# ShenhanQian/GaussianAvatars

Measured on AMD Instinct MI355X. Metric: frames/sec fwd+bwd @100k SH-3 splats 802x550, higher is better.
Workload: dtype f32; 1 GPU; BASELINE configs[2]: 100000 mesh-bound SH-3 splats (synthetic stand-in for media/306), 802x550 (HxW), select_mesh_by_timestep + render + L1-vs-white + backward, no optimiser step; splats=100000, width=550, height=802, sh_degree=3, scene=ellipsoid, splat_order=morton (io.spatial_sort: the loaders' default), num_rendered=2322054, num_binned=1851307, tile_culling=True, binding=fused, parallelism=one process, one GPU, 300 frames in turn; no collective

## Files before the change

### gaussianavatars_amd/csrc/gsr_backward.hip

```cpp
#include "gsr_device.h"

#include <hip/amd_detail/amd_hip_unsafe_atomics.h>

namespace gsr {

__device__ __forceinline__ float swap32_add(float a, float b)
{
    const auto r = __builtin_amdgcn_permlane32_swap(__float_as_uint(a), __float_as_uint(b), false, false);
    return __uint_as_float(r[0]) + __uint_as_float(r[1]);
}
__device__ __forceinline__ float swap16_add(float a, float b)
{
    const auto r = __builtin_amdgcn_permlane16_swap(__float_as_uint(a), __float_as_uint(b), false, false);
    return __uint_as_float(r[0]) + __uint_as_float(r[1]);
}
__device__ __forceinline__ float bank_merge(float keep, float take, const int bank_mask_sel)
{
    return bank_mask_sel == 0xA
               ? __int_as_float(__builtin_amdgcn_update_dpp(__float_as_int(keep), __float_as_int(take), 0xE4, 0xf, 0xA, false))
               : __int_as_float(__builtin_amdgcn_update_dpp(__float_as_int(keep), __float_as_int(take), 0xE4, 0xf, 0xC, false));
}
__device__ __forceinline__ float row_sum4(float a, float b, float c, float d)
{
    a += dpp_f<0x141, 0xf>(a);
// ... 358 lines not shown
        const int j = hi - 1 - lane;
        const bool valid = lane < CH && j < nq;
        const uint32_t idx = qp[valid ? j : nq - 1];
        const float4 r0 = grec[3 * (size_t)idx + 0], r1 = grec[3 * (size_t)idx + 1], r2 = grec[3 * (size_t)idx + 2];
        const float xq = r0.x - fqx0, yq = r0.y - fqy0;
        const float cA = r0.z, cB = r0.w, cC = r1.x;
        const float op = valid ? r2.z : 0.f;
        const float cr = r1.z, cgn = r1.w, cb = r2.x;
        const int jrec = valid ? j : 0x7fffffff;
        const unsigned long long act = __ballot(last_pix > lo);
        const bool more = lo > seg_lo;
        f2 a0 = {0.f, 0.f}, a1 = a0, a2 = a0, a3 = a0, a4 = a0, a5 = a0, a6 = a0, a7 = a0, a8 = a0;

        for (int r = 0; r < 8; ++r) {
            const uint32_t rm = (uint32_t)(act >> (8 * r)) & 0xFFu;
            if (!rm) continue;
            const float dy = yq - (float)r;
            const float Bdy = cB * dy, Cdy2 = (cC * dy) * dy;
#ifndef GSR_EXP_NO_ROW_SUMS
            f2 rs0 = {0.f, 0.f}, rs1 = rs0, rs2 = rs0;
#endif
#pragma unroll
            for (int h = 0; h < 2; ++h) {
                if (!((rm >> (4 * h)) & 0xFu)) continue;
                const f4* tp = reinterpret_cast<const f4*>(tab + (r * 4 + 2 * h) * 12);
                f4 t[2][3];
#pragma unroll
                for (int e = 0; e < 2; ++e)
#pragma unroll
                    for (int k = 0; k < 3; ++k) t[e][k] = tp[3 * e + k];
                f2 dx[2], a0m[2], al[2], rv[2], R[2], Tj[2], cg[2], aT[2], Pw[2];
#pragma unroll
                for (int e = 0; e < 2; ++e) {
                    const float c0 = (float)(4 * h + 2 * e);
                    dx[e] = f2{xq - c0, xq - (c0 + 1.0f)};
                    const f2 pw = (cA * dx[e] + Bdy) * dx[e] + Cdy2;
                    const f2 G = {__builtin_amdgcn_exp2f(pw.x), __builtin_amdgcn_exp2f(pw.y)};
                    const f2 araw = op * G;
                    const int l0 = __float_as_int(t[e][2].z), l1 = __float_as_int(t[e][2].w);
#ifdef GSR_EXP_HI_TEST
                    a0m[e].x = (l0 > jrec && pw.x <= 0.0f && araw.x >= 1.0f / 255.0f) ? araw.x : 0.0f;
                    a0m[e].y = (l1 > jrec && pw.y <= 0.0f && araw.y >= 1.0f / 255.0f) ? araw.y : 0.0f;
#else
                    a0m[e].x = (l0 > jrec && araw.x >= 1.0f / 255.0f) ? araw.x : 0.0f;
                    a0m[e].y = (l1 > jrec && araw.y >= 1.0f / 255.0f) ? araw.y : 0.0f;
#endif
                    al[e] = f2{__builtin_fminf(0.99f, a0m[e].x), __builtin_fminf(0.99f, a0m[e].y)};
                    const f2 om = 1.0f - al[e];
                    rv[e] = f2{__builtin_amdgcn_rcpf(om.x), __builtin_amdgcn_rcpf(om.y)};
                    R[e] = rv[e];
                }
#ifndef GSR_EXP_RP_NOSCAN
                GSR_SCAN4("v_mul_f32_dpp", R[0].x, R[0].y, R[1].x, R[1].y);
#endif
#pragma unroll
                for (int e = 0; e < 2; ++e) {
                    const f2 Te = {t[e][0].x, t[e][0].y};
                    const f2 g0 = {t[e][1].x, t[e][1].y}, g1 = {t[e][1].z, t[e][1].w}, g2 = {t[e][2].x, t[e][2].y};
                    Tj[e] = Te * R[e];
                    cg[e] = cr * g0 + (cgn * g1 + cb * g2);
                    aT[e] = al[e] * Tj[e];
                    Pw[e] = aT[e] * cg[e];
                }
#ifndef GSR_EXP_RP_NOSCAN
                GSR_SCAN4("v_add_f32_dpp", Pw[0].x, Pw[0].y, Pw[1].x, Pw[1].y);
#endif
#pragma unroll
                for (int e = 0; e < 2; ++e) {
                    const f2 Sx = {t[e][0].z, t[e][0].w};
                    const f2 g0 = {t[e][1].x, t[e][1].y}, g1 = {t[e][1].z, t[e][1].w}, g2 = {t[e][2].x, t[e][2].y};
                    const f2 dLda = ((Tj[e] * cg[e] - Pw[e]) - Sx) * rv[e];
                    const f2 tq = a0m[e] * dLda;
                    a0 += aT[e] * g0;
                    a1 += aT[e] * g1;
                    a2 += aT[e] * g2;
#ifndef GSR_EXP_NO_ROW_SUMS
                    const f2 ax = tq * dx[e];
                    rs0 += tq;
                    rs1 += ax;
                    rs2 += ax * dx[e];
#else
                    const f2 ax = tq * dx[e], ay = tq * dy;
                    a3 += ax;
                    a4 += ay;
                    a5 += ax * dx[e];
                    a6 += ax * dy;
                    a7 += ay * dy;
                    a8 += tq;
#endif
                    if (more) {
                        const float T0 = __int_as_float(__builtin_amdgcn_readlane(__float_as_int(Tj[e].x), CH - 1));
                        const float T1 = __int_as_float(__builtin_amdgcn_readlane(__float_as_int(Tj[e].y), CH - 1));
                        const float S0 = __int_as_float(__builtin_amdgcn_readlane(__float_as_int(Pw[e].x), CH - 1)) + Sx.x;
                        const float S1 = __int_as_float(__builtin_amdgcn_readlane(__float_as_int(Pw[e].y), CH - 1)) + Sx.y;
                        if (lane == 0) {
                            float* up = tab + (r * 4 + 2 * h + e) * 12;
                            up[0] = T0; up[1] = T1; up[2] = S0; up[3] = S1;
                        }
                    }
                }
            }
#ifndef GSR_EXP_NO_ROW_SUMS
            a3 += rs1;
            a4 += rs0 * dy;
            a5 += rs2;
            a6 += rs1 * dy;
            a7 += rs0 * (dy * dy);
            a8 += rs0;
#endif
        }
#ifndef GSR_EXP_RP_NOATOMIC
        {
            const float v[9] = {a0.x + a0.y, a1.x + a1.y, a2.x + a2.y, a3.x + a3.y, a4.x + a4.y, a5.x + a5.y, a6.x + a6.y, a7.x + a7.y, a8.x + a8.y};
#pragma unroll
            for (int c = 0; c < 9; ++c) xs[9 * lane + c] = v[c];
#pragma unroll
            for (int i = 0; i < (CH + 6) / 7; ++i) {
                const int rl7 = (lane * 7282) >> 16;
                const int c = lane - 9 * rl7;
                const int rl = 7 * i + rl7;
                const float val = xs[63 * i + lane];
                const uint32_t rid = (uint32_t)__builtin_amdgcn_ds_bpermute(rl << 2, (int)idx);
                const bool live = lane < 63 && rl < CH && (hi - 1 - rl) < nq;
#ifdef GSR_EXP_RP_PLAINSTORE
                if (live && val == 12345.678f) acc[(size_t)GSR_ACC_STRIDE * rid + c] = val;
#else
                if (live && val != 0.f) unsafeAtomicAdd(acc + (size_t)GSR_ACC_STRIDE * rid + c, val);
#endif
            }
        }
#endif
        if (!more) break;
        hi = lo;
    }
    }
}

template __global__ void k_render_bwd_rp<1>(Settings, const uint32_t*, const uint32_t*, const float4*, const uint32_t*, const float*, const uint32_t*, const float*, float*, const float*,
                                             const float4*, int, unsigned long long, const unsigned long long*, const uint32_t*);
template __global__ void k_render_bwd_rp<2>(Settings, const uint32_t*, const uint32_t*, const float4*, const uint32_t*, const float*, const uint32_t*, const float*, float*, const float*,
                                             const float4*, int, unsigned long long, const unsigned long long*, const uint32_t*);
template __global__ void k_render_bwd_rp<4>(Settings, const uint32_t*, const uint32_t*, const float4*, const uint32_t*, const float*, const uint32_t*, const float*, float*, const float*,
                                             const float4*, int, unsigned long long, const unsigned long long*, const uint32_t*);


__global__ __launch_bounds__(GSR_PREBWD_ROWS) void k_preprocess_bwd(Settings s, PreBwdArgs a)
{
    const int i = blockIdx.x * blockDim.x + threadIdx.x;
    const int M = a.M;
    __shared__ float sh_lds[GSR_PREBWD_ROWS * GSR_SH_MAX_STRIDE];
    const bool sh_staged = !a.use_precomp_color && a.dL_dsh != nullptr && M <= 16;
    const int first = blockIdx.x * GSR_PREBWD_ROWS, rows = min(GSR_PREBWD_ROWS, a.P - first);
    const int sh_stride = sh_row_stride(M);
    if (sh_staged) {
        if (a.shs_rest) {
            sh_rows_load<GSR_PREBWD_ROWS>(sh_lds, a.shs, first, rows, 3, sh_stride, 0, (int)threadIdx.x);
            sh_rows_load<GSR_PREBWD_ROWS>(sh_lds, a.shs_rest, first, rows, 3 * (M - 1), sh_stride, 3, (int)threadIdx.x);
        } else {
            sh_rows_load<GSR_PREBWD_ROWS>(sh_lds, a.shs, first, rows, 3 * M, sh_stride, 0, (int)threadIdx.x);
        }
        __syncthreads();
    }
    if (i < a.P) {
    float dmean[3] = {0.f, 0.f, 0.f};
    float gcov[6] = {0.f, 0.f, 0.f, 0.f, 0.f, 0.f};
    float dscale[3] = {0.f, 0.f, 0.f};
    float drot[4] = {0.f, 0.f, 0.f, 0.f};
    float gcol[3] = {0.f, 0.f, 0.f};
    float g2x = 0.f, g2y = 0.f, gop = 0.f;
    const bool vis = a.radii[i] > 0;
    float* gsh = a.dL_dsh ? (sh_staged ? sh_lds + (int)threadIdx.x * sh_row_stride(M) : a.dL_dsh + (size_t)3 * M * i) : nullptr;

    if (vis) {
        float4 q0, q1, q2;
        if (s.deterministic) {
            long long* ai = a.acc64 + (size_t)GSR_ACC64_STRIDE * i;
            const int ex = __float_as_int(a.grec[3 * (size_t)i + 2].y), back = gmax_exponent(*a.gmax) - GSR_FIXED_BITS;
            float f[9];
#pragma unroll
            for (int k = 0; k < 9; ++k) { f[k] = __builtin_ldexpf((float)ai[k], back + ((k >= 5 && k <= 7) ? (ex >> 8) : (ex & 0xFF))); ai[k] = 0ll; }
            q0 = make_float4(f[0], f[1], f[2], f[3]); q1 = make_float4(f[4], f[5], f[6], f[7]); q2 = make_float4(f[8], 0.f, 0.f, 0.f);
        } else {
            float4* ac4 = (float4*)(a.acc + (size_t)GSR_ACC_STRIDE * i);
            q0 = ac4[0]; q1 = ac4[1]; q2 = ac4[2];
            const float4 z = make_float4(0.f, 0.f, 0.f, 0.f);
            ac4[0] = z; ac4[1] = z; ac4[2] = z;
        }
        gcol[0] = q0.x; gcol[1] = q0.y; gcol[2] = q0.z;
        g2x = -0.5f * (float)s.W * q0.w; g2y = -0.5f * (float)s.H * q1.x;
        const float gA = -0.5f * q1.y, gB = -0.5f * q1.z, gC = -0.5f * q1.w;
        gop = q2.x;
        const float* vm = s.viewmatrix;
        const float* proj = s.projmatrix;
        const int W = s.W, H = s.H;
        const float fx = (float)W / (2.0f * s.tanfovx), fy = (float)H / (2.0f * s.tanfovy);
        float mx = a.means3D[3 * i], my = a.means3D[3 * i + 1], mz = a.means3D[3 * i + 2];
        if (a.bound.binding) {
            const long long bface = bound_face(a.bound, i);
            float w[3];
            bindm::world_xyz(a.bound.fR + 9 * bface, a.bound.fs[bface], a.bound.fc + 3 * bface, mx, my, mz, w);
            mx = w[0]; my = w[1]; mz = w[2];
        }
        const float* c6 = a.cov3D + 6 * i;

        if (!a.use_precomp_color) {
            float shr[48];
            {
                const float* row = sh_staged ? sh_lds + (int)threadIdx.x * sh_row_stride(M) : a.shs + (size_t)3 * M * i;
#pragma unroll
                for (int k = 0; k < 48; ++k) shr[k] = k < 3 * M ? row[k] : 0.f;
            }
            const float* sh = shr;
            const int deg = s.sh_degree;
            const float d0 = mx - s.campos[0], d1 = my - s.campos[1], d2 = mz - s.campos[2];
            const float sum2 = d0 * d0 + d1 * d1 + d2 * d2;
            const float inv_len = 1.0f / sqrtf(sum2);
            const float x = d0 * inv_len, y = d1 * inv_len, z = d2 * inv_len;
            const uint32_t cl = a.clamped[i];
            float ddir[3] = {0.f, 0.f, 0.f};
            const float xx = x * x, yy = y * y, zz = z * z, xy_ = x * y, yz = y * z, xz = x * z;
            const int ncoef = (deg + 1) * (deg + 1);
#pragma unroll
            for (int c = 0; c < 3; ++c) {
                const float g = ((cl >> c) & 1u) ? 0.f : gcol[c];
                float dxs = 0.f, dys = 0.f, dzs = 0.f;
                gsh[0 + c] = kC0 * g;
                if (deg > 0) {
                    gsh[3 + c] = -kC1 * y * g;
                    gsh[6 + c] = kC1 * z * g;
                    gsh[9 + c] = -kC1 * x * g;
                    dxs = -kC1 * sh[9 + c];
                    dys = -kC1 * sh[3 + c];
                    dzs = kC1 * sh[6 + c];
                    if (deg > 1) {
                        gsh[12 + c] = kC2_0 * xy_ * g;
                        gsh[15 + c] = kC2_1 * yz * g;
                        gsh[18 + c] = kC2_2 * (2.f * zz - xx - yy) * g;
                        gsh[21 + c] = kC2_3 * xz * g;
                        gsh[24 + c] = kC2_4 * (xx - yy) * g;
                        dxs += kC2_0 * y * sh[12 + c] + kC2_2 * 2.f * -x * sh[18 + c] + kC2_3 * z * sh[21 + c] + kC2_4 * 2.f * x * sh[24 + c];
                        dys += kC2_0 * x * sh[12 + c] + kC2_1 * z * sh[15 + c] + kC2_2 * 2.f * -y * sh[18 + c] + kC2_4 * 2.f * -y * sh[24 + c];
                        dzs += kC2_1 * y * sh[15 + c] + kC2_2 * 2.f * 2.f * z * sh[18 + c] + kC2_3 * x * sh[21 + c];
                        if (deg > 2) {
                            gsh[27 + c] = kC3_0 * y * (3.f * xx - yy) * g;
                            gsh[30 + c] = kC3_1 * xy_ * z * g;
                            gsh[33 + c] = kC3_2 * y * (4.f * zz - xx - yy) * g;
                            gsh[36 + c] = kC3_3 * z * (2.f * zz - 3.f * xx - 3.f * yy) * g;
                            gsh[39 + c] = kC3_4 * x * (4.f * zz - xx - yy) * g;
                            gsh[42 + c] = kC3_5 * z * (xx - yy) * g;
                            gsh[45 + c] = kC3_6 * x * (xx - 3.f * yy) * g;
                            dxs += kC3_0 * sh[27 + c] * 3.f * 2.f * xy_ + kC3_1 * sh[30 + c] * yz + kC3_2 * sh[33 + c] * -2.f * xy_ +
                                   kC3_3 * sh[36 + c] * -3.f * 2.f * xz + kC3_4 * sh[39 + c] * (-3.f * xx + 4.f * zz - yy) +
                                   kC3_5 * sh[42 + c] * 2.f * xz + kC3_6 * sh[45 + c] * 3.f * (xx - yy);
                            dys += kC3_0 * sh[27 + c] * 3.f * (xx - yy) + kC3_1 * sh[30 + c] * xz +
                                   kC3_2 * sh[33 + c] * (-3.f * yy + 4.f * zz - xx) + kC3_3 * sh[36 + c] * -3.f * 2.f * yz +
                                   kC3_4 * sh[39 + c] * -2.f * xy_ + kC3_5 * sh[42 + c] * -2.f * yz + kC3_6 * sh[45 + c] * -3.f * 2.f * xy_;
                            dzs += kC3_1 * sh[30 + c] * xy_ + kC3_2 * sh[33 + c] * 4.f * 2.f * yz +
                                   kC3_3 * sh[36 + c] * 3.f * (2.f * zz - xx - yy) + kC3_4 * sh[39 + c] * 4.f * 2.f * xz +
                                   kC3_5 * sh[42 + c] * (xx - yy);
                        }
                    }
                }
                ddir[0] += dxs * g;
                ddir[1] += dys * g;
                ddir[2] += dzs * g;
            }
            for (int k = 3 * ncoef; k < 3 * M; ++k) gsh[k] = 0.f;
            const float invsum32 = 1.0f / sqrtf(sum2 * sum2 * sum2);
            dmean[0] += ((sum2 - d0 * d0) * ddir[0] - d1 * d0 * ddir[1] - d2 * d0 * ddir[2]) * invsum32;
            dmean[1] += (-d0 * d1 * ddir[0] + (sum2 - d1 * d1) * ddir[1] - d2 * d1 * ddir[2]) * invsum32;
            dmean[2] += (-d0 * d2 * ddir[0] - d1 * d2 * ddir[1] + (sum2 - d2 * d2) * ddir[2]) * invsum32;
        }

        float t0 = vm[0] * mx + vm[4] * my + vm[8] * mz + vm[12];
        float t1 = vm[1] * mx + vm[5] * my + vm[9] * mz + vm[13];
        const float t2 = vm[2] * mx + vm[6] * my + vm[10] * mz + vm[14];
        const float limx = 1.3f * s.tanfovx, limy = 1.3f * s.tanfovy;
        const float txtz = t0 / t2, tytz = t1 / t2;
        t0 = sel_min(limx, sel_max(-limx, txtz)) * t2;
        t1 = sel_min(limy, sel_max(-limy, tytz)) * t2;
        const float x_grad_mul = (txtz < -limx || txtz > limx) ? 0.f : 1.f;
        const float y_grad_mul = (tytz < -limy || tytz > limy) ? 0.f : 1.f;
        const float J00 = fx / t2, J02 = -(fx * t0) / (t2 * t2), J11 = fy / t2, J12 = -(fy * t1) / (t2 * t2);
        float A[2][3];
#pragma unroll
        for (int j = 0; j < 3; ++j) {
            A[0][j] = J00 * vm[4 * j + 0] + J02 * vm[4 * j + 2];
            A[1][j] = J11 * vm[4 * j + 1] + J12 * vm[4 * j + 2];
        }
        const float V[3][3] = {{c6[0], c6[1], c6[2]}, {c6[1], c6[3], c6[4]}, {c6[2], c6[4], c6[5]}};
        float AV[2][3];
#pragma unroll
        for (int r = 0; r < 2; ++r)
#pragma unroll
            for (int j = 0; j < 3; ++j) AV[r][j] = A[r][0] * V[0][j] + A[r][1] * V[1][j] + A[r][2] * V[2][j];
        const float ca = AV[0][0] * A[0][0] + AV[0][1] * A[0][1] + AV[0][2] * A[0][2] + 0.3f;
        const float cb = AV[0][0] * A[1][0] + AV[0][1] * A[1][1] + AV[0][2] * A[1][2];
        const float cc = AV[1][0] * A[1][0] + AV[1][1] * A[1][1] + AV[1][2] * A[1][2] + 0.3f;
        const float denom = ca * cc - cb * cb;
        if (s.fast_blend) {
            const float det_inv = 1.f / denom;
            const float kA = cc * det_inv, kB = -cb * det_inv, kC = ca * det_inv;
            g2x = -0.5f * (float)s.W * (kA * q0.w + kB * q1.x);
            g2y = -0.5f * (float)s.H * (kC * q1.x + kB * q0.w);
            const float opac = a.grec[3 * (size_t)i + 2].z;
            gop = opac > 0.f ? q2.x / opac : 0.f;
        }
        const float denom2inv = 1.0f / ((denom * denom) + 0.0000001f);
        float dL_da = 0.f, dL_db = 0.f, dL_dc = 0.f;
        if (denom2inv != 0.f) {
            dL_da = denom2inv * (-cc * cc * gA + 2.f * cb * cc * gB + (denom - ca * cc) * gC);
            dL_dc = denom2inv * (-ca * ca * gC + 2.f * ca * cb * gB + (denom - ca * cc) * gA);
            dL_db = denom2inv * 2.f * (cb * cc * gA - (denom + 2.f * cb * cb) * gB + ca * cb * gC);
            gcov[0] = A[0][0] * A[0][0] * dL_da + A[0][0] * A[1][0] * dL_db + A[1][0] * A[1][0] * dL_dc;
            gcov[3] = A[0][1] * A[0][1] * dL_da + A[0][1] * A[1][1] * dL_db + A[1][1] * A[1][1] * dL_dc;
            gcov[5] = A[0][2] * A[0][2] * dL_da + A[0][2] * A[1][2] * dL_db + A[1][2] * A[1][2] * dL_dc;
            gcov[1] = 2.f * A[0][0] * A[0][1] * dL_da + (A[0][0] * A[1][1] + A[0][1] * A[1][0]) * dL_db + 2.f * A[1][0] * A[1][1] * dL_dc;
            gcov[2] = 2.f * A[0][0] * A[0][2] * dL_da + (A[0][0] * A[1][2] + A[0][2] * A[1][0]) * dL_db + 2.f * A[1][0] * A[1][2] * dL_dc;
            gcov[4] = 2.f * A[0][2] * A[0][1] * dL_da + (A[0][1] * A[1][2] + A[0][2] * A[1][1]) * dL_db + 2.f * A[1][1] * A[1][2] * dL_dc;
        }
        float dA[2][3];
#pragma unroll
        for (int j = 0; j < 3; ++j) {
            const float a0v = A[0][0] * V[j][0] + A[0][1] * V[j][1] + A[0][2] * V[j][2];
            const float a1v = A[1][0] * V[j][0] + A[1][1] * V[j][1] + A[1][2] * V[j][2];
            dA[0][j] = 2.f * a0v * dL_da + a1v * dL_db;
            dA[1][j] = 2.f * a1v * dL_dc + a0v * dL_db;
        }
        const float dJ00 = vm[0] * dA[0][0] + vm[4] * dA[0][1] + vm[8] * dA[0][2];
        const float dJ02 = vm[2] * dA[0][0] + vm[6] * dA[0][1] + vm[10] * dA[0][2];
        const float dJ11 = vm[1] * dA[1][0] + vm[5] * dA[1][1] + vm[9] * dA[1][2];
        const float dJ12 = vm[2] * dA[1][0] + vm[6] * dA[1][1] + vm[10] * dA[1][2];
        const float tz = 1.f / t2, tz2 = tz * tz, tz3 = tz2 * tz;
        const float dtx = x_grad_mul * -fx * tz2 * dJ02;
        const float dty = y_grad_mul * -fy * tz2 * dJ12;
        const float dtz = -fx * tz2 * dJ00 - fy * tz2 * dJ11 + (2.f * fx * t0) * tz3 * dJ02 + (2.f * fy * t1) * tz3 * dJ12;
        dmean[0] += vm[0] * dtx + vm[1] * dty + vm[2] * dtz;
        dmean[1] += vm[4] * dtx + vm[5] * dty + vm[6] * dtz;
        dmean[2] += vm[8] * dtx + vm[9] * dty + vm[10] * dtz;

        const float hw = proj[3] * mx + proj[7] * my + proj[11] * mz + proj[15];
        const float m_w = 1.0f / (hw + 0.0000001f);
        const float mul1 = (proj[0] * mx + proj[4] * my + proj[8] * mz + proj[12]) * m_w * m_w;
        const float mul2 = (proj[1] * mx + proj[5] * my + proj[9] * mz + proj[13]) * m_w * m_w;
        dmean[0] += (proj[0] * m_w - proj[3] * mul1) * g2x + (proj[1] * m_w - proj[3] * mul2) * g2y;
        dmean[1] += (proj[4] * m_w - proj[7] * mul1) * g2x + (proj[5] * m_w - proj[7] * mul2) * g2y;
        dmean[2] += (proj[8] * m_w - proj[11] * mul1) * g2x + (proj[9] * m_w - proj[11] * mul2) * g2y;

        if (!a.use_precomp_cov) {
            float4 q = reinterpret_cast<const float4*>(a.rotations)[i];
            float ws[3] = {a.scales[3 * i], a.scales[3 * i + 1], a.scales[3 * i + 2]};
            if (a.bound.binding) {
                const long long bface = bound_face(a.bound, i);
                q = bindm::world_rotation(reinterpret_cast<const float4*>(a.bound.fq)[bface], q);
                const float bscale = a.bound.fs[bface];
#pragma unroll
                for (int k = 0; k < 3; ++k) ws[k] = bindm::world_scaling(ws[k], bscale);
            } else if (a.bound.leaves) {
                q = bindm::unit_rotation(q);
#pragma unroll
                for (int k = 0; k < 3; ++k) ws[k] = bindm::world_scaling(ws[k], 1.f);
            }
            const float r = q.x, x = q.y, y = q.z, z = q.w;
            float R[3][3];
            R[0][0] = 1.f - 2.f * (y * y + z * z);
            R[0][1] = 2.f * (x * y - r * z);
            R[0][2] = 2.f * (x * z + r * y);
            R[1][0] = 2.f * (x * y + r * z);
            R[1][1] = 1.f - 2.f * (x * x + z * z);
            R[1][2] = 2.f * (y * z - r * x);
            R[2][0] = 2.f * (x * z - r * y);
            R[2][1] = 2.f * (y * z + r * x);
            R[2][2] = 1.f - 2.f * (x * x + y * y);
            const float mod = s.scale_modifier;
            const float sc[3] = {mod * ws[0], mod * ws[1], mod * ws[2]};
            const float gS[3][3] = {{gcov[0], 0.5f * gcov[1], 0.5f * gcov[2]},
                                    {0.5f * gcov[1], gcov[3], 0.5f * gcov[4]},
                                    {0.5f * gcov[2], 0.5f * gcov[4], gcov[5]}};
            float dR[3][3];
#pragma unroll
            for (int k = 0; k < 3; ++k) {
                float dMk[3];
#pragma unroll
                for (int j = 0; j < 3; ++j)
                    dMk[j] = 2.0f * sc[k] * (R[0][k] * gS[0][j] + R[1][k] * gS[1][j] + R[2][k] * gS[2][j]);
                dscale[k] = (s.exact_scale_grad ? mod : 1.0f) * (R[0][k] * dMk[0] + R[1][k] * dMk[1] + R[2][k] * dMk[2]);
#pragma unroll
                for (int j = 0; j < 3; ++j) dR[j][k] = sc[k] * dMk[j];
            }
            drot[0] = 2.f * z * (dR[1][0] - dR[0][1]) + 2.f * y * (dR[0][2] - dR[2][0]) + 2.f * x * (dR[2][1] - dR[1][2]);
            drot[1] = 2.f * y * (dR[0][1] + dR[1][0]) + 2.f * z * (dR[0][2] + dR[2][0]) + 2.f * r * (dR[2][1] - dR[1][2]) - 4.f * x * (dR[2][2] + dR[1][1]);
            drot[2] = 2.f * x * (dR[0][1] + dR[1][0]) + 2.f * r * (dR[0][2] - dR[2][0]) + 2.f * z * (dR[1][2] + dR[2][1]) - 4.f * y * (dR[2][2] + dR[0][0]);
            drot[3] = 2.f * r * (dR[1][0] - dR[0][1]) + 2.f * x * (dR[0][2] + dR[2][0]) + 2.f * y * (dR[1][2] + dR[2][1]) - 4.f * z * (dR[1][1] + dR[0][0]);
        }
    } else if (gsh) {
        for (int k = 0; k < 3 * M; ++k) gsh[k] = 0.f;
    }

    if (a.bound.binding) {
        const long long bface = bound_face(a.bound, i);
        float Rf[9];
#pragma unroll
        for (int k = 0; k < 9; ++k) Rf[k] = a.bound.fR[9 * bface + k];
        const float xl[3] = {a.means3D[3 * i], a.means3D[3 * i + 1], a.means3D[3 * i + 2]};
        const float ls[3] = {a.scales ? a.scales[3 * i] : 0.f, a.scales ? a.scales[3 * i + 1] : 0.f, a.scales ? a.scales[3 * i + 2] : 0.f};
        const float4 ql = a.rotations ? reinterpret_cast<const float4*>(a.rotations)[i] : make_float4(1.f, 0.f, 0.f, 0.f);
        float dx[3], dls[3], acc[BINDM_ROW];
        float4 dq;
        bindm::bind_backward(Rf, a.bound.fs[bface], reinterpret_cast<const float4*>(a.bound.fq)[bface], xl, ls, ql, dmean, dscale,
                             make_float4(drot[0], drot[1], drot[2], drot[3]), dx, dls, &dq, acc);
#pragma unroll
        for (int k = 0; k < 3; ++k) { dmean[k] = dx[k]; dscale[k] = dls[k]; }
        drot[0] = dq.x; drot[1] = dq.y; drot[2] = dq.z; drot[3] = dq.w;
        const float o = bindm::sigmoid(a.opacities[i]);
        gop = gop * o * (1.f - o);
        float4* row = reinterpret_cast<float4*>(a.bound.rows + (size_t)BINDM_ROW * a.bound.slot[i]);
#pragma unroll
        for (int k = 0; k < BINDM_ROW / 4; ++k) row[k] = make_float4(acc[4 * k], acc[4 * k + 1], acc[4 * k + 2], acc[4 * k + 3]);
    }
    else if (a.bound.leaves) {
        if (a.scales) {
#pragma unroll
            for (int k = 0; k < 3; ++k) dscale[k] *= bindm::world_scaling(a.scales[3 * i + k], 1.f);
        }
        if (a.rotations) {
            const float4 dq = bindm::unit_rotation_backward(reinterpret_cast<const float4*>(a.rotations)[i], make_float4(drot[0], drot[1], drot[2], drot[3]));
            drot[0] = dq.x; drot[1] = dq.y; drot[2] = dq.z; drot[3] = dq.w;
        }
        const float o = bindm::sigmoid(a.opacities[i]);
        gop = gop * o * (1.f - o);
    }
#pragma unroll
    for (int k = 0; k < 3; ++k) a.dL_dmeans3D[3 * i + k] = dmean[k];
    a.dL_dmeans2D[3 * i + 0] = g2x;
    a.dL_dmeans2D[3 * i + 1] = g2y;
    a.dL_dmeans2D[3 * i + 2] = 0.f;
    if (a.dL_dcolors) {
#pragma unroll
        for (int k = 0; k < 3; ++k) a.dL_dcolors[3 * i + k] = gcol[k];
    }
    a.dL_dopacity[i] = gop;
    if (a.dL_dcov3D) {
#pragma unroll
        for (int k = 0; k < 6; ++k) a.dL_dcov3D[6 * i + k] = gcov[k];
    }
    if (a.dL_dscales) {
#pragma unroll
        for (int k = 0; k < 3; ++k) a.dL_dscales[3 * i + k] = dscale[k];
    }
    if (a.dL_drotations) reinterpret_cast<float4*>(a.dL_drotations)[i] = make_float4(drot[0], drot[1], drot[2], drot[3]);
    }
    if (sh_staged) {
        __syncthreads();
        if (a.shs_rest) {
            sh_rows_store<GSR_PREBWD_ROWS>(sh_lds, a.dL_dsh, first, rows, 3, sh_stride, 0, (int)threadIdx.x);
            sh_rows_store<GSR_PREBWD_ROWS>(sh_lds, a.dL_dsh_rest, first, rows, 3 * (M - 1), sh_stride, 3, (int)threadIdx.x);
        } else {
            sh_rows_store<GSR_PREBWD_ROWS>(sh_lds, a.dL_dsh, first, rows, 3 * M, sh_stride, 0, (int)threadIdx.x);
        }
    }
}

}
```

### gaussianavatars_amd/csrc/gsr_device.h

```cpp
#pragma once
#include <hip/hip_runtime.h>
#include <stdint.h>

#include "../../include/gsr.h"

#define GSR_WAVE 64
#define GSR_TILE_PIX (GSR_BLOCK_X * GSR_BLOCK_Y)
#define GSR_SORT_LDS_KEYS 8192
#define GSR_SORT_XL_KEYS 16384
#define GSR_SORT_SMALL_KEYS 2048
#define GSR_ACC_STRIDE 16
#define GSR_ACC64_STRIDE 10
#define GSR_FIXED_BITS 58
#define GSR_LDS_HIST_TILES 40960
#define GSR_RANK_MAX_BUCKETS 4096
#define GSR_RANK_HIST_TILES (GSR_LDS_HIST_TILES - GSR_RANK_MAX_BUCKETS)
#define GSR_RANK_BANDS 24
#define GSR_RANK_MAX_BANDS 32
#define GSR_RANK_BAND_CHUNK 256
#define GSR_RANK_IDX_BITS 28
#define GSR_RANK_MAX_SPLATS 262144
#define GSR_RANK_TILE_THREADS 512
#define GSR_RANK_WINDOW 4096
#ifndef GSR_RANK_GROUP
// ... 136 lines not shown
struct Reach {
    float px, py, A, B, C, tau, nBiC, nBiA;
    int mode;
};
__device__ __forceinline__ Reach reach_of(float px, float py, float A, float B, float C, float opacity)
{
    Reach r;
    r.px = px; r.py = py; r.A = A; r.B = B; r.C = C;
    r.tau = 0.f; r.nBiC = 0.f; r.nBiA = 0.f;
    if (!(opacity * 255.0f >= 1.0f)) { r.mode = 2; return r; }
    r.tau = logf(255.0f * opacity) * 1.0001f + 1e-3f;
    if (!(A > 0.f && C > 0.f && (A * C - B * B) > 0.f)) { r.mode = 1; return r; }
    r.nBiC = -B / C;
    r.nBiA = -B / A;
    r.mode = 0;
    return r;
}
__device__ __forceinline__ bool rect_reach(const Reach& r, float x0, float y0, float w, float h)
{
    if (r.mode) return r.mode == 1;
    const float a0 = r.px - (x0 + w), a1 = r.px - x0;
    const float b0 = r.py - (y0 + h), b1 = r.py - y0;
    const bool in_x = a0 <= 0.f && a1 >= 0.f, in_y = b0 <= 0.f && b1 >= 0.f;
    if (in_x && in_y) return true;
    const float a = a0 > 0.f ? a0 : a1;
    const float b = b0 > 0.f ? b0 : b1;
    const float dyv = fminf(fmaxf(r.nBiC * a, b0), b1);
    const float qv = 0.5f * (r.A * a * a + 2.f * r.B * a * dyv + r.C * dyv * dyv);
    const float dxh = fminf(fmaxf(r.nBiA * b, a0), a1);
    const float qh = 0.5f * (r.A * dxh * dxh + 2.f * r.B * dxh * b + r.C * b * b);
    const float big = 3.0e38f;
    const float mn = fminf(in_x ? big : qv, in_y ? big : qh);
    return mn * 0.999f - 1e-3f <= r.tau;
}

struct Span {
    float px, py, B, det, twoTA, A, dyr;
    int mode;
};
__device__ __forceinline__ Span span_of(const Reach& r)
{
    Span s;
    s.px = r.px; s.py = r.py; s.B = r.B; s.mode = r.mode;
    s.det = 0.f; s.twoTA = 0.f; s.A = 0.f; s.dyr = 0.f;
    if (r.mode) return s;
    const float T = (r.tau + 1e-3f) / 0.999f;
    s.det = r.A * r.C - r.B * r.B;
    s.twoTA = 2.f * T * r.A;
    s.A = r.A;
    s.dyr = r.nBiC * sqrtf(2.f * T * r.C / s.det);
    if (!(fabsf(s.dyr) < 1e15f && s.twoTA < 1e30f && s.A > 1e-30f && s.A < 1e30f && s.det > 0.f)) s.mode = 1;
    return s;
}
struct Band {
    float dl, dr, Bbl, Bbr;
    int any;
};
__device__ __forceinline__ Band band_of(const Span& s, float y0)
{
    Band e;
    e.dl = e.dr = e.Bbl = e.Bbr = 0.f;
    if (s.mode) { e.any = s.mode == 1 ? 2 : 0; return e; }
    const float b0 = y0 - s.py, b1 = b0 + 7.f;
    const float br = fminf(fmaxf(s.dyr, b0), b1), bl = fminf(fmaxf(-s.dyr, b0), b1);
    e.dr = s.twoTA - s.det * br * br;
    e.dl = s.twoTA - s.det * bl * bl;
    e.Bbr = s.B * br;
    e.Bbl = s.B * bl;
    e.any = (e.dr >= 0.f && e.dl >= 0.f) ? 1 : 0;
    return e;
}
__device__ __forceinline__ bool band_hit(const Band& e, const Span& s, float x0)
{
    const float tl = (s.px - 1e-2f - (x0 + 7.f)) * s.A - e.Bbl;
    const float tr = (x0 - s.px - 1e-2f) * s.A + e.Bbr;
    const bool hit = (tl <= 0.f || e.dl >= tl * tl) && (tr <= 0.f || e.dr >= tr * tr);
    return e.any == 2 || (e.any == 1 && hit);
}

__device__ __forceinline__ void snug_rect(const Reach& r, int& minx, int& miny, int& maxx, int& maxy, uint32_t& n)
{
    if (r.mode == 1 || n == 0) return;
    if (r.mode == 2) { n = 0; return; }
    const float det = r.A * r.C - r.B * r.B;
    const float k = 2.f * r.tau / det;
    const float xr = sqrtf(k * r.C) * 1.001f + 1e-2f, yr = sqrtf(k * r.A) * 1.001f + 1e-2f;
    if (!(xr < 1e9f && yr < 1e9f)) return;
    const float fx = (float)GSR_BLOCK_X, fy = (float)GSR_BLOCK_Y;
    const int lox = (int)ceilf((r.px - xr - (fx - 1.f)) / fx), hix = (int)floorf((r.px + xr) / fx) + 1;
    const int loy = (int)ceilf((r.py - yr - (fy - 1.f)) / fy), hiy = (int)floorf((r.py + yr) / fy) + 1;
    minx = max(minx, lox); maxx = min(maxx, hix);
    miny = max(miny, loy); maxy = min(maxy, hiy);
    n = (maxx > minx && maxy > miny) ? (uint32_t)((maxx - minx) * (maxy - miny)) : 0u;
}

__device__ __forceinline__ uint32_t quadrant_mask_of(const Span& s, float ox, float oy)
{
    uint32_t m = 0u;
#pragma unroll
    for (int by = 0; by < 2; ++by) {
        const float y0 = by ? oy + 8.f : oy;
        const float b0 = y0 - s.py, b1 = b0 + 7.f;
        const float br = fminf(fmaxf(s.dyr, b0), b1), bl = fminf(fmaxf(-s.dyr, b0), b1);
        const float dr = s.twoTA - s.det * br * br;
        const float dl = s.twoTA - s.det * bl * bl;
        const float Bbr = s.B * br;
        const float Bbl = s.B * bl;
        const uint32_t any = (uint32_t)(dr >= 0.f) & (uint32_t)(dl >= 0.f);
#pragma unroll
        for (int bx = 0; bx < 2; ++bx) {
            const float x0 = bx ? ox + 8.f : ox;
            const float tl = (s.px - 1e-2f - (x0 + 7.f)) * s.A - Bbl;
            const float tr = (x0 - s.px - 1e-2f) * s.A + Bbr;
            const uint32_t hit = ((uint32_t)(tl <= 0.f) | (uint32_t)(dl >= tl * tl)) & ((uint32_t)(tr <= 0.f) | (uint32_t)(dr >= tr * tr)) & any;
            m |= hit << (2 * by + bx);
        }
    }
    return s.mode == 1 ? 15u : (s.mode == 2 ? 0u : m);
}
__device__ __forceinline__ uint32_t quadrant_mask(float2 p, float4 co, float ox, float oy)
{
    return quadrant_mask_of(span_of(reach_of(p.x, p.y, co.x, co.y, co.z, co.w)), ox, oy);
}

template <typename F>
__device__ __forceinline__ void for_each_tile(int minx, int miny, int maxx, int maxy, uint32_t n, int gx, F f,
                                              uint32_t payload0, uint32_t payload1)
{
    constexpr uint32_t SMALL = 16;
    if (n > 0 && n <= SMALL) {
        for (int y = miny; y < maxy; ++y)
            for (int x = minx; x < maxx; ++x) f((uint32_t)(y * gx + x), payload0, payload1);
    }
    uint64_t big = __ballot(n > SMALL);
    const int lane = lane_id();
    while (big) {
        const int src = __builtin_ctzll(big);
        big &= big - 1;
        const int bminx = __builtin_amdgcn_readlane(minx, src);
        const int bminy = __builtin_amdgcn_readlane(miny, src);
        const int bmaxx = __builtin_amdgcn_readlane(maxx, src);
        const uint32_t bn = (uint32_t)__builtin_amdgcn_readlane((int)n, src);
        const uint32_t p0 = (uint32_t)__builtin_amdgcn_readlane((int)payload0, src);
        const uint32_t p1 = (uint32_t)__builtin_amdgcn_readlane((int)payload1, src);
        const uint32_t w = (uint32_t)(bmaxx - bminx);
        for (uint32_t k = (uint32_t)lane; k < bn; k += GSR_WAVE) {
            const uint32_t y = (uint32_t)bminy + k / w;
            const uint32_t x = (uint32_t)bminx + k % w;
            f(y * (uint32_t)gx + x, p0, p1);
        }
    }
}

#define GSR_SH_ROWS 256
#ifndef GSR_PREBWD_ROWS
#define GSR_PREBWD_ROWS 208
#endif
#define GSR_SH_MAX_STRIDE 49
__device__ __forceinline__ int sh_row_stride(int M) { return (3 * M) | 1; }

template <int NT = GSR_SH_ROWS>
__device__ __forceinline__ void sh_rows_load(float* __restrict__ lds, const float* __restrict__ src, int first, int rows, int w, int stride,
                                             int col0, int tid)
{
    const int total = rows * w;
    const float* base = src + (size_t)first * w;
    if ((total & 3) == 0 && ((((size_t)first * w) & 3) == 0)) {
        const float4* b4 = reinterpret_cast<const float4*>(base);
        for (int f = tid * 4; f < total; f += NT * 4) {
            const float4 v = b4[f >> 2];
            int r = f / w, c = f - r * w;
            const float e[4] = {v.x, v.y, v.z, v.w};
#pragma unroll
            for (int k = 0; k < 4; ++k) {
                lds[r * stride + col0 + c] = e[k];
                if (++c == w) { c = 0; ++r; }
            }
        }
    } else {
        for (int f = tid; f < total; f += NT) {
            const int r = f / w, c = f - r * w;
            lds[r * stride + col0 + c] = base[f];
        }
    }
}

template <int NT = GSR_SH_ROWS>
__device__ __forceinline__ void sh_rows_store(const float* __restrict__ lds, float* __restrict__ dst, int first, int rows, int w, int stride,
                                              int col0, int tid)
{
    const int total = rows * w;
    float* base = dst + (size_t)first * w;
    if ((total & 3) == 0 && ((((size_t)first * w) & 3) == 0)) {
        float4* b4 = reinterpret_cast<float4*>(base);
        for (int f = tid * 4; f < total; f += NT * 4) {
            int r = f / w, c = f - r * w;
            float e[4];
#pragma unroll
            for (int k = 0; k < 4; ++k) {
                e[k] = lds[r * stride + col0 + c];
                if (++c == w) { c = 0; ++r; }
            }
            b4[f >> 2] = make_float4(e[0], e[1], e[2], e[3]);
        }
    } else {
        for (int f = tid; f < total; f += NT) {
            const int r = f / w, c = f - r * w;
            base[f] = lds[r * stride + col0 + c];
        }
    }
}

#define GSR_STAT_SLOTS 32
struct BinStatSlot {
    uint32_t nvis, dmin_inv, dmax_bits, pad0;
    unsigned long long binned_tiles, rect_total;
    uint32_t pad1[8];
};
struct BinHeader {
    unsigned long long total;
    unsigned long long rect_total;
    uint32_t nvis;
    uint32_t dmin_inv;
    uint32_t dmax_bits;
    uint32_t dmin_bits;
    unsigned long long binned_tiles;
    uint32_t band_total[GSR_RANK_MAX_BANDS];
    uint32_t chunk_imbalance;
    uint32_t pad[21];
    BinStatSlot slot[GSR_STAT_SLOTS];
};
static_assert(sizeof(BinHeader) == 256 + 64 * GSR_STAT_SLOTS, "header layout is part of include/gsr.h");

#define GSR_WALK_MASKS 2
struct QBinArgs {
    int Q, gx;
    uint32_t chunks;
    BinHeader* __restrict__ hdr;
    const float4* __restrict__ brec;
    const uint32_t* __restrict__ order;
    uint32_t* __restrict__ qhist;
    const uint32_t* __restrict__ qprefix;
    const uint32_t* __restrict__ qstart;
    uint32_t* __restrict__ qpos;
    unsigned long long* __restrict__ qmask;
    unsigned long long capacity;
};

struct BoundDev {
    int leaves;
    const void* __restrict__ binding;
    int is64;
    const float* __restrict__ fR;
    const float* __restrict__ fs;
    const float* __restrict__ fc;
    const float* __restrict__ fq;
    const int* __restrict__ slot;
    float* __restrict__ rows;
};
__device__ __forceinline__ long long bound_face(const BoundDev& b, int i)
{
    return b.is64 ? reinterpret_cast<const long long*>(b.binding)[i] : (long long)reinterpret_cast<const int*>(b.binding)[i];
}

struct PreprocessArgs {
    int P, M;
    const float* __restrict__ means3D;
    const float* __restrict__ shs;
    const float* __restrict__ shs_rest;
    const float* __restrict__ colors_precomp;
    const float* __restrict__ opacities;
    const float* __restrict__ scales;
    const float* __restrict__ rotations;
    const float* __restrict__ cov3D_precomp;
    int32_t* __restrict__ radii;
    float* __restrict__ depths;
    float4* __restrict__ grec;
    float* __restrict__ cov3D;
    ushort4* __restrict__ rect;
    uint32_t* __restrict__ tiles_touched;
    uint8_t* __restrict__ clamped;
    uint8_t* __restrict__ visible;
    float4* __restrict__ acc;
    float4* __restrict__ acc64;
    uint32_t* __restrict__ tile_count;
    uint32_t* __restrict__ units;
    unsigned long long* __restrict__ rect_total;
    int tiles;
    float4* __restrict__ brec;
    BinHeader* __restrict__ hdr;
    uint32_t* __restrict__ bcount;
    int nb;
    uint32_t* __restrict__ bcursor;
    uint4* __restrict__ pstat;
    ushort4* __restrict__ srect;
    float4* __restrict__ sspan;
    int cull;
    BoundDev bound;
};

struct PreBwdArgs {
    int P, M;
    const float* __restrict__ means3D;
    const float* __restrict__ shs;
    const float* __restrict__ shs_rest;
    const float* __restrict__ scales;
    const float* __restrict__ rotations;
    const float* __restrict__ cov3D;
    const int32_t* __restrict__ radii;
    const uint8_t* __restrict__ clamped;
    float* __restrict__ acc;
    long long* __restrict__ acc64;
    const uint32_t* __restrict__ gmax;
    const float4* __restrict__ grec;
    int use_precomp_cov, use_precomp_color;
    float* __restrict__ dL_dmeans3D;
    float* __restrict__ dL_dmeans2D;
    float* __restrict__ dL_dsh;
    float* __restrict__ dL_dsh_rest;
    float* __restrict__ dL_dcolors;
    float* __restrict__ dL_dopacity;
    float* __restrict__ dL_dscales;
    float* __restrict__ dL_drotations;
    float* __restrict__ dL_dcov3D;
    BoundDev bound;
    const float* __restrict__ opacities;
};

__global__ void k_preprocess(Settings s, PreprocessArgs a);
__global__ void k_tile_scan(int tiles, const uint32_t* tile_count, uint32_t* tile_start, uint32_t* tile_cursor, uint2* ranges,
                            uint32_t* tile_order, unsigned long long* total_dev, unsigned long long* mailbox, unsigned long long seq, unsigned long long post_capacity);
template <bool CULL>
__global__ void k_count(int P, int gx, int tiles, const ushort4* rect, const uint32_t* tiles_touched, const float4* grec, uint32_t* tile_count,
                        unsigned long long* rect_total, uint32_t* block_hist);
template <bool CULL>
__global__ void k_scatter(int P, int gx, int tiles, const float* depths, const ushort4* rect, const uint32_t* tiles_touched, const float4* grec,
                          const uint32_t* tile_start, uint32_t* tile_cursor, unsigned long long* keys,
                          unsigned long long capacity, const unsigned long long* total_dev, const uint32_t* block_hist);
template <int KEYS, int THREADS>
__global__ void k_tile_sort(uint32_t n_lo, uint32_t n_hi, int gx, const uint32_t* tile_order, const uint32_t* tile_count, const uint32_t* tile_start, unsigned long long* keys,
// ... 115 lines not shown
```

Baseline: 3860 frames/s.

## Prefetch per-splat inputs into registers before SH LDS staging in preprocess backward

```diff
diff --git a/gaussianavatars_amd/csrc/gsr_backward.hip b/gaussianavatars_amd/csrc/gsr_backward.hip
--- a/gaussianavatars_amd/csrc/gsr_backward.hip
+++ b/gaussianavatars_amd/csrc/gsr_backward.hip
@@ -534,37 +534,85 @@
     const bool sh_staged = !a.use_precomp_color && a.dL_dsh != nullptr && M <= 16;
     const int first = blockIdx.x * GSR_PREBWD_ROWS, rows = min(GSR_PREBWD_ROWS, a.P - first);
     const int sh_stride = sh_row_stride(M);
+    const bool live = i < a.P, bound = a.bound.binding != nullptr;
+    long long bface = 0;
+    if (live && bound) bface = bound_face(a.bound, i);
+    ShRowsRound<GSR_PREBWD_ROWS, 3> sh_dc;
+    ShRowsRound<GSR_PREBWD_ROWS, 3 * 16> sh_main;
     if (sh_staged) {
         if (a.shs_rest) {
-            sh_rows_load<GSR_PREBWD_ROWS>(sh_lds, a.shs, first, rows, 3, sh_stride, 0, (int)threadIdx.x);
-            sh_rows_load<GSR_PREBWD_ROWS>(sh_lds, a.shs_rest, first, rows, 3 * (M - 1), sh_stride, 3, (int)threadIdx.x);
+            sh_dc.issue(a.shs, first, rows, 3, (int)threadIdx.x);
+            sh_main.issue(a.shs_rest, first, rows, 3 * (M - 1), (int)threadIdx.x);
         } else {
-            sh_rows_load<GSR_PREBWD_ROWS>(sh_lds, a.shs, first, rows, 3 * M, sh_stride, 0, (int)threadIdx.x);
+            sh_main.issue(a.shs, first, rows, 3 * M, (int)threadIdx.x);
+        }
+    }
+    int rad = 0, slot = 0;
+    uint32_t cl = 0;
+    float m3[3] = {0.f, 0.f, 0.f}, ls3[3] = {0.f, 0.f, 0.f}, c6[6] = {0.f, 0.f, 0.f, 0.f, 0.f, 0.f}, oraw = 0.f;
+    float4 qraw = make_float4(1.f, 0.f, 0.f, 0.f), g2 = make_float4(0.f, 0.f, 0.f, 0.f);
+    float4 q0 = make_float4(0.f, 0.f, 0.f, 0.f), q1 = q0, q2 = q0;
+    float Rf[9] = {0.f, 0.f, 0.f, 0.f, 0.f, 0.f, 0.f, 0.f, 0.f}, fsv = 1.f, fcv[3] = {0.f, 0.f, 0.f};
+    float4 fqv = make_float4(1.f, 0.f, 0.f, 0.f);
+    if (live) {
+        rad = a.radii[i];
+        if (!s.deterministic) {
+            const float4* ac4 = (const float4*)(a.acc + (size_t)GSR_ACC_STRIDE * i);
+            q0 = ac4[0]; q1 = ac4[1]; q2 = ac4[2];
+        }
+#pragma unroll
+        for (int k = 0; k < 3; ++k) m3[k] = a.means3D[3 * i + k];
+#pragma unroll
+        for (int k = 0; k < 6; ++k) c6[k] = a.cov3D[6 * i + k];
+        if (!a.use_precomp_cov || bound) {
+            if (a.rotations) qraw = reinterpret_cast<const float4*>(a.rotations)[i];
+            if (a.scales) {
+#pragma unroll
+                for (int k = 0; k < 3; ++k) ls3[k] = a.scales[3 * i + k];
+            }
+        }
+        if (!a.use_precomp_color) cl = a.clamped[i];
+        if (s.deterministic || s.fast_blend) g2 = a.grec[3 * (size_t)i + 2];
+        if (bound || a.bound.leaves) oraw = a.opacities[i];
+        if (bound) {
+            slot = a.bound.slot[i];
+#pragma unroll
+            for (int k = 0; k < 9; ++k) Rf[k] = a.bound.fR[9 * bface + k];
+            fsv = a.bound.fs[bface];
+#pragma unroll
+            for (int k = 0; k < 3; ++k) fcv[k] = a.bound.fc[3 * bface + k];
+            fqv = reinterpret_cast<const float4*>(a.bound.fq)[bface];
+        }
+    }
+    if (sh_staged) {
+        if (a.shs_rest) {
+            sh_dc.commit(sh_lds, a.shs, first, rows, 3, sh_stride, 0, (int)threadIdx.x);
+            sh_main.commit(sh_lds, a.shs_rest, first, rows, 3 * (M - 1), sh_stride, 3, (int)threadIdx.x);
+        } else {
+            sh_main.commit(sh_lds, a.shs, first, rows, 3 * M, sh_stride, 0, (int)threadIdx.x);
         }
         __syncthreads();
     }
-    if (i < a.P) {
+    if (live) {
     float dmean[3] = {0.f, 0.f, 0.f};
     float gcov[6] = {0.f, 0.f, 0.f, 0.f, 0.f, 0.f};
     float dscale[3] = {0.f, 0.f, 0.f};
     float drot[4] = {0.f, 0.f, 0.f, 0.f};
     float gcol[3] = {0.f, 0.f, 0.f};
     float g2x = 0.f, g2y = 0.f, gop = 0.f;
-    const bool vis = a.radii[i] > 0;
+    const bool vis = rad > 0;
     float* gsh = a.dL_dsh ? (sh_staged ? sh_lds + (int)threadIdx.x * sh_row_stride(M) : a.dL_dsh + (size_t)3 * M * i) : nullptr;
 
     if (vis) {
-        float4 q0, q1, q2;
         if (s.deterministic) {
             long long* ai = a.acc64 + (size_t)GSR_ACC64_STRIDE * i;
-            const int ex = __float_as_int(a.grec[3 * (size_t)i + 2].y), back = gmax_exponent(*a.gmax) - GSR_FIXED_BITS;
+            const int ex = __float_as_int(g2.y), back = gmax_exponent(*a.gmax) - GSR_FIXED_BITS;
             float f[9];
 #pragma unroll
             for (int k = 0; k < 9; ++k) { f[k] = __builtin_ldexpf((float)ai[k], back + ((k >= 5 && k <= 7) ? (ex >> 8) : (ex & 0xFF))); ai[k] = 0ll; }
             q0 = make_float4(f[0], f[1], f[2], f[3]); q1 = make_float4(f[4], f[5], f[6], f[7]); q2 = make_float4(f[8], 0.f, 0.f, 0.f);
         } else {
             float4* ac4 = (float4*)(a.acc + (size_t)GSR_ACC_STRIDE * i);
-            q0 = ac4[0]; q1 = ac4[1]; q2 = ac4[2];
             const float4 z = make_float4(0.f, 0.f, 0.f, 0.f);
             ac4[0] = z; ac4[1] = z; ac4[2] = z;
         }
@@ -576,14 +624,12 @@
         const float* proj = s.projmatrix;
         const int W = s.W, H = s.H;
         const float fx = (float)W / (2.0f * s.tanfovx), fy = (float)H / (2.0f * s.tanfovy);
-        float mx = a.means3D[3 * i], my = a.means3D[3 * i + 1], mz = a.means3D[3 * i + 2];
-        if (a.bound.binding) {
-            const long long bface = bound_face(a.bound, i);
+        float mx = m3[0], my = m3[1], mz = m3[2];
+        if (bound) {
             float w[3];
-            bindm::world_xyz(a.bound.fR + 9 * bface, a.bound.fs[bface], a.bound.fc + 3 * bface, mx, my, mz, w);
+            bindm::world_xyz(Rf, fsv, fcv, mx, my, mz, w);
             mx = w[0]; my = w[1]; mz = w[2];
         }
-        const float* c6 = a.cov3D + 6 * i;
 
         if (!a.use_precomp_color) {
             float shr[48];
@@ -598,7 +644,6 @@
             const float sum2 = d0 * d0 + d1 * d1 + d2 * d2;
             const float inv_len = 1.0f / sqrtf(sum2);
             const float x = d0 * inv_len, y = d1 * inv_len, z = d2 * inv_len;
-            const uint32_t cl = a.clamped[i];
             float ddir[3] = {0.f, 0.f, 0.f};
             const float xx = x * x, yy = y * y, zz = z * z, xy_ = x * y, yz = y * z, xz = x * z;
             const int ncoef = (deg + 1) * (deg + 1);
@@ -685,7 +730,7 @@
             const float kA = cc * det_inv, kB = -cb * det_inv, kC = ca * det_inv;
             g2x = -0.5f * (float)s.W * (kA * q0.w + kB * q1.x);
             g2y = -0.5f * (float)s.H * (kC * q1.x + kB * q0.w);
-            const float opac = a.grec[3 * (size_t)i + 2].z;
+            const float opac = g2.z;
             gop = opac > 0.f ? q2.x / opac : 0.f;
         }
         const float denom2inv = 1.0f / ((denom * denom) + 0.0000001f);
@@ -730,12 +775,11 @@
         dmean[2] += (proj[8] * m_w - proj[11] * mul1) * g2x + (proj[9] * m_w - proj[11] * mul2) * g2y;
 
         if (!a.use_precomp_cov) {
-            float4 q = reinterpret_cast<const float4*>(a.rotations)[i];
-            float ws[3] = {a.scales[3 * i], a.scales[3 * i + 1], a.scales[3 * i + 2]};
-            if (a.bound.binding) {
-                const long long bface = bound_face(a.bound, i);
-                q = bindm::world_rotation(reinterpret_cast<const float4*>(a.bound.fq)[bface], q);
-                const float bscale = a.bound.fs[bface];
+            float4 q = qraw;
+            float ws[3] = {ls3[0], ls3[1], ls3[2]};
+            if (bound) {
+                q = bindm::world_rotation(fqv, q);
+                const float bscale = fsv;
 #pragma unroll
                 for (int k = 0; k < 3; ++k) ws[k] = bindm::world_scaling(ws[k], bscale);
             } else if (a.bound.leaves) {
@@ -779,37 +823,30 @@
         for (int k = 0; k < 3 * M; ++k) gsh[k] = 0.f;
     }
 
-    if (a.bound.binding) {
-        const long long bface = bound_face(a.bound, i);
-        float Rf[9];
-#pragma unroll
-        for (int k = 0; k < 9; ++k) Rf[k] = a.bound.fR[9 * bface + k];
-        const float xl[3] = {a.means3D[3 * i], a.means3D[3 * i + 1], a.means3D[3 * i + 2]};
-        const float ls[3] = {a.scales ? a.scales[3 * i] : 0.f, a.scales ? a.scales[3 * i + 1] : 0.f, a.scales ? a.scales[3 * i + 2] : 0.f};
-        const float4 ql = a.rotations ? reinterpret_cast<const float4*>(a.rotations)[i] : make_float4(1.f, 0.f, 0.f, 0.f);
+    if (bound) {
         float dx[3], dls[3], acc[BINDM_ROW];
         float4 dq;
-        bindm::bind_backward(Rf, a.bound.fs[bface], reinterpret_cast<const float4*>(a.bound.fq)[bface], xl, ls, ql, dmean, dscale,
+        bindm::bind_backward(Rf, fsv, fqv, m3, ls3, qraw, dmean, dscale,
                              make_float4(drot[0], drot[1], drot[2], drot[3]), dx, dls, &dq, acc);
 #pragma unroll
         for (int k = 0; k < 3; ++k) { dmean[k] = dx[k]; dscale[k] = dls[k]; }
         drot[0] = dq.x; drot[1] = dq.y; drot[2] = dq.z; drot[3] = dq.w;
-        const float o = bindm::sigmoid(a.opacities[i]);
+        const float o = bindm::sigmoid(oraw);
         gop = gop * o * (1.f - o);
-        float4* row = reinterpret_cast<float4*>(a.bound.rows + (size_t)BINDM_ROW * a.bound.slot[i]);
+        float4* row = reinterpret_cast<float4*>(a.bound.rows + (size_t)BINDM_ROW * slot);
 #pragma unroll
         for (int k = 0; k < BINDM_ROW / 4; ++k) row[k] = make_float4(acc[4 * k], acc[4 * k + 1], acc[4 * k + 2], acc[4 * k + 3]);
     }
     else if (a.bound.leaves) {
         if (a.scales) {
 #pragma unroll
-            for (int k = 0; k < 3; ++k) dscale[k] *= bindm::world_scaling(a.scales[3 * i + k], 1.f);
+            for (int k = 0; k < 3; ++k) dscale[k] *= bindm::world_scaling(ls3[k], 1.f);
         }
         if (a.rotations) {
-            const float4 dq = bindm::unit_rotation_backward(reinterpret_cast<const float4*>(a.rotations)[i], make_float4(drot[0], drot[1], drot[2], drot[3]));
+            const float4 dq = bindm::unit_rotation_backward(qraw, make_float4(drot[0], drot[1], drot[2], drot[3]));
             drot[0] = dq.x; drot[1] = dq.y; drot[2] = dq.z; drot[3] = dq.w;
         }
-        const float o = bindm::sigmoid(a.opacities[i]);
+        const float o = bindm::sigmoid(oraw);
         gop = gop * o * (1.f - o);
     }
 #pragma unroll
diff --git a/gaussianavatars_amd/csrc/gsr_device.h b/gaussianavatars_amd/csrc/gsr_device.h
--- a/gaussianavatars_amd/csrc/gsr_device.h
+++ b/gaussianavatars_amd/csrc/gsr_device.h
@@ -312,40 +312,58 @@
     }
 }
 
-#define GSR_SH_ROWS 256
 #ifndef GSR_PREBWD_ROWS
-#define GSR_PREBWD_ROWS 208
+#define GSR_PREBWD_ROWS 64
 #endif
 #define GSR_SH_MAX_STRIDE 49
 __device__ __forceinline__ int sh_row_stride(int M) { return (3 * M) | 1; }
 
-template <int NT = GSR_SH_ROWS>
-__device__ __forceinline__ void sh_rows_load(float* __restrict__ lds, const float* __restrict__ src, int first, int rows, int w, int stride,
-                                             int col0, int tid)
-{
-    const int total = rows * w;
-    const float* base = src + (size_t)first * w;
-    if ((total & 3) == 0 && ((((size_t)first * w) & 3) == 0)) {
-        const float4* b4 = reinterpret_cast<const float4*>(base);
-        for (int f = tid * 4; f < total; f += NT * 4) {
-            const float4 v = b4[f >> 2];
-            int r = f / w, c = f - r * w;
-            const float e[4] = {v.x, v.y, v.z, v.w};
+template <int NT, int MAXW>
+struct ShRowsRound {
+    static constexpr int IT = (MAXW + 3) / 4;
+    float4 v[IT];
+    bool vec;
+    __device__ __forceinline__ void issue(const float* __restrict__ src, int first, int rows, int w, int tid)
+    {
+        const int total = rows * w;
+        vec = (total & 3) == 0 && ((((size_t)first * w) & 3) == 0);
+        if (vec) {
+            const float4* b4 = reinterpret_cast<const float4*>(src + (size_t)first * w);
 #pragma unroll
-            for (int k = 0; k < 4; ++k) {
-                lds[r * stride + col0 + c] = e[k];
-                if (++c == w) { c = 0; ++r; }
+            for (int k = 0; k < IT; ++k) {
+                const int f = (tid + NT * k) * 4;
+                v[k] = f < total ? b4[f >> 2] : make_float4(0.f, 0.f, 0.f, 0.f);
             }
         }
-    } else {
-        for (int f = tid; f < total; f += NT) {
-            const int r = f / w, c = f - r * w;
-            lds[r * stride + col0 + c] = base[f];
+    }
+    __device__ __forceinline__ void commit(float* __restrict__ lds, const float* __restrict__ src, int first, int rows, int w, int stride, int col0, int tid) const
+    {
+        const int total = rows * w;
+        if (vec) {
+#pragma unroll
+            for (int k = 0; k < IT; ++k) {
+                const int f = (tid + NT * k) * 4;
+                if (f < total) {
+                    int r = f / w, c = f - r * w;
+                    const float e[4] = {v[k].x, v[k].y, v[k].z, v[k].w};
+#pragma unroll
+                    for (int j = 0; j < 4; ++j) {
+                        lds[r * stride + col0 + c] = e[j];
+                        if (++c == w) { c = 0; ++r; }
+                    }
+                }
+            }
+        } else {
+            const float* base = src + (size_t)first * w;
+            for (int f = tid; f < total; f += NT) {
+                const int r = f / w, c = f - r * w;
+                lds[r * stride + col0 + c] = base[f];
+            }
         }
     }
-}
-
-template <int NT = GSR_SH_ROWS>
+};
+
+template <int NT>
 __device__ __forceinline__ void sh_rows_store(const float* __restrict__ lds, float* __restrict__ dst, int first, int rows, int w, int stride,
                                               int col0, int tid)
 {
```

Result: slower. 3760 frames/s (-2.6%).
